# george-gca/sr-pytorch-lightning

Measured on AMD Instinct MI355X. Metric: SR training throughput, LR patches/s (48x48 LR x4, fwd+bwd+Adam), higher is better.
Workload: dtype bf16; 1 GPU; edsr_baseline x4, 48x48 LR patches, batch 256/GPU, train step (L1 + Adam); global_batch=256, parallelism=dp1, hip_graph=full

## Files before the change

include/srk.h:

```cpp
#ifndef SRK_H
#define SRK_H

#include <stdint.h>

#ifdef __cplusplus
extern "C" {
#endif

typedef void* srk_stream_t;

enum { SRK_BF16 = 0, SRK_F16 = 1, SRK_F32 = 2 };

enum {
  SRK_E_BADARG = -1,
  SRK_E_NODEV = -2
};

enum {
  SRK_OUT_NHWC = 0,
  SRK_OUT_NHWC_PS = 1,
  SRK_OUT_PLANAR = 2
};

typedef struct {
// ... 175 lines not shown
  const float* src; void* dst; int dst_pitch, dst_coff;
  int N, C, H, W;
  int Cstore; int ps_r; float scale; int dtype;
} srk_to_nhwc_args;
int srk_nchw_to_nhwc(const srk_to_nhwc_args* a, srk_stream_t stream);

typedef struct {
  const void* src; int src_pitch, src_coff; float* dst;
  int N, C, H, W; int dtype;
} srk_to_nchw_args;
int srk_nhwc_to_nchw(const srk_to_nchw_args* a, srk_stream_t stream);

int srk_ca_splits(int N, int HW);
typedef struct {
  const void* t; int t_pitch, t_coff;
  const void* u; int u_pitch, u_coff;
  float* sums;
  int N, HW, C; int dtype;
} srk_ca_pool_args;
int srk_ca_pool(const srk_ca_pool_args* a, srk_stream_t stream);

typedef struct {
  const void* t; int t_pitch, t_coff;
  const void* res; int res_pitch, res_coff;
  const float* sums;
  const float* w1; const float* b1; const float* w2; const float* b2;
  float* s_out; float* z_out;
  void* out; int out_pitch, out_coff;
  int N, HW, C, Cr; int dtype;
  int sums_rows;
} srk_ca_apply_args;
int srk_ca_apply(const srk_ca_apply_args* a, srk_stream_t stream);

typedef struct {
  const void* g; int g_pitch, g_coff;
  const float* gsum;
  const float* sums; const float* s; const float* z;
  const float* w1; const float* w2;
  float* dw1; float* db1; float* dw2; float* db2;
  void* gt; int gt_pitch, gt_coff;
  int N, HW, C, Cr; int dtype;
  int sums_rows, gsum_rows;
} srk_ca_bwd_args;
int srk_ca_bwd_apply(const srk_ca_bwd_args* a, srk_stream_t stream);
typedef struct { const float* src; float* dst; int n; int k; } srk_rowsum_job;
int srk_rowsum_group(const srk_rowsum_job* table_dev, int njobs, int max_k, srk_stream_t stream);

typedef struct {
  const uint8_t* lr; const uint8_t* hr;
  int lr_h, lr_w, hr_h, hr_w;
  int top, left;
  int rot;
  int hflip, vflip;
} srk_patch_desc;
typedef struct {
  const srk_patch_desc* table; int N; int C; int patch_lr; int scale;
  float* lr_out;
  float* hr_out;
} srk_patch_args;
int srk_sample_patches(const srk_patch_args* a, srk_stream_t stream);

typedef struct {
  const float* sr; const float* hr;
  int N, C, H, W;
  int luma;
  int shave;
  double* sse;
} srk_sse_args;
int srk_image_sse(const srk_sse_args* a, srk_stream_t stream);

typedef struct srk_l1_args {
  const float* sr;
  const float* hr;
  long long n;
  signed char* sign;
  double* partial;
  const float* gout;
  float scale;
  float* grad;
} srk_l1_args;
int srk_l1_blocks(long long n);
int srk_l1_loss_fwd(const srk_l1_args* a, srk_stream_t stream);
int srk_l1_loss_bwd(const srk_l1_args* a, srk_stream_t stream);
int srk_l1_loss_mean(const double* partial, int nb, long long n, float* out, srk_stream_t stream);

#define SRK_FLIP_TABLE_FLOATS 176
#define SRK_FLIP_ADJ_CHANNELS 7
typedef struct srk_flip_args {
  const float* sr;
  const float* hr;
  int N, H, W;
  const float* table;
  double* partial;
  float* err;
  float* adj;
  const float* gout;
  float scale;
  float* grad;
} srk_flip_args;
int srk_flip_blocks(int N, int H, int W);
int srk_flip_fwd(const srk_flip_args* a, srk_stream_t stream);
int srk_flip_bwd(const srk_flip_args* a, srk_stream_t stream);
int srk_flip_mean(const double* partial, int nb, long long n, float* out, srk_stream_t stream);

typedef struct srk_haarpsi_args {
  const float* sr;
  const float* hr;
  int N, C, H, W;
  double* partial;
  float* planes;
  float* stats;
  float* loss;
  float* index;
  const float* gout;
  float* grad;
} srk_haarpsi_args;
int srk_haarpsi_tiles(int N, int H, int W);
int srk_haarpsi_fwd(const srk_haarpsi_args* a, srk_stream_t stream);
int srk_haarpsi_finalize(const srk_haarpsi_args* a, srk_stream_t stream);
int srk_haarpsi_bwd(const srk_haarpsi_args* a, srk_stream_t stream);

typedef struct srk_ssim_loss_args {
  const float* sr;
  const float* hr;
  int N, C, H, W;
  double* partial;
  float* loss;
  const float* gout;
  float* grad;
} srk_ssim_loss_args;
int srk_ssim_loss_tiles(int N, int C, int H, int W);
int srk_ssim_loss_fwd(const srk_ssim_loss_args* a, srk_stream_t stream);
int srk_ssim_loss_finalize(const srk_ssim_loss_args* a, srk_stream_t stream);
int srk_ssim_loss_bwd(const srk_ssim_loss_args* a, srk_stream_t stream);

typedef struct srk_ms_ssim_loss_args {
  const float* sr;
  const float* hr;
  int N, C, H, W;
  float* workspace;
  double* partials;
  float* table;
  float* loss;
  const float* gout;
  float* gwork;
  float* grad;
} srk_ms_ssim_loss_args;
long long srk_ms_ssim_loss_workspace_bytes(int N, int C, int H, int W);
int srk_ms_ssim_loss_tiles(int N, int C, int H, int W, int* first);
int srk_ms_ssim_loss_fwd(const srk_ms_ssim_loss_args* a, srk_stream_t stream);
int srk_ms_ssim_loss_finalize(const srk_ms_ssim_loss_args* a, srk_stream_t stream);
int srk_ms_ssim_loss_bwd(const srk_ms_ssim_loss_args* a, srk_stream_t stream);

typedef struct srk_gmsd_args {
  const float* sr;
  const float* hr;
  int N, C, H, W;
  double* partial;
  float* stats;
  float* loss;
  const float* gout;
  float* grad;
} srk_gmsd_args;
int srk_gmsd_tiles(int N, int C, int H, int W);
int srk_gmsd_fwd(const srk_gmsd_args* a, srk_stream_t stream);
int srk_gmsd_finalize(const srk_gmsd_args* a, srk_stream_t stream);
// ... 225 lines not shown
```

sr-pytorch-lightning_amd/_lib.py:

```python
import ctypes as C
import os

_HERE = os.path.dirname(os.path.abspath(__file__))
EXACT_RELU = os.environ.get("SRK_EXACT_RELU") == "1"
LIB_PATH = os.environ.get("SRK_LIB_PATH") or os.path.join(_HERE, "libsrk_gfx950_exact.so" if EXACT_RELU else "libsrk_gfx950.so")

SRK_BF16, SRK_F16, SRK_F32 = 0, 1, 2
OUT_NHWC, OUT_NHWC_PS, OUT_PLANAR = 0, 1, 2

_p, _i, _f = C.c_void_p, C.c_int, C.c_float


class PackArgs(C.Structure):
    _fields_ = [("w", _p), ("bias", _p), ("wpk", _p), ("bias_pk", _p),
                ("Cout", _i), ("Cin", _i), ("KH", _i), ("KW", _i),
                ("KinP", _i), ("CoutP", _i), ("dgrad", _i), ("ps_r", _i), ("dtype", _i), ("rows_layout", _i)]


class ConvArgs(C.Structure):
    _fields_ = [("x", _p), ("x_pitch", _i), ("x_coff", _i), ("x_ps", _i),
                ("N", _i), ("H", _i), ("W", _i), ("Cin", _i),
                ("wpk", _p), ("bias", _p), ("CoutP", _i), ("Cout", _i), ("KH", _i), ("KW", _i),
                ("relu", _i), ("scale", _f),
                ("res", _p), ("res_pitch", _i), ("res_coff", _i),
# ... 97 lines not shown
                ("dwp", _p), ("dbp", _p), ("nslabs", _i), ("dtype", _i), ("cout_real", _i)]


class WgradFinArgs(C.Structure):
    _fields_ = [("dwp", _p), ("dbp", _p), ("nslabs", _i), ("dw", _p), ("db", _p),
                ("Cout", _i), ("Cin", _i), ("KH", _i), ("KW", _i), ("CinP", _i), ("CoutP", _i),
                ("ps_r", _i), ("scale", _f), ("accumulate", _i)]


class ProjArgs(C.Structure):
    _fields_ = [("x", _p), ("x_pitch", _i), ("out", _p), ("out_pitch", _i), ("wpk", _p), ("bias", _p),
                ("N", _i), ("H", _i), ("W", _i), ("dtype", _i), ("slope", _p), ("slope_stride", _i), ("pre", _p), ("pre_pitch", _i)]


class ProjPackJob(C.Structure):
    _fields_ = [("w4", _p), ("wpk", _p)]


class ProjWgradArgs(C.Structure):
    _fields_ = [("xh", _p), ("xh_pitch", _i), ("g", _p), ("g_pitch", _i), ("scratch", _p), ("dw", _p), ("accumulate", _i),
                ("N", _i), ("H", _i), ("W", _i), ("dtype", _i), ("db", _p), ("bias_side", _i), ("db_accumulate", _i)]


class UnfoldArgs(C.Structure):
    _fields_ = [("x", _p), ("sub", _p), ("dst", _p), ("dst_pitch", _i), ("dst_coff", _i),
                ("N", _i), ("Cin", _i), ("H", _i), ("W", _i), ("KH", _i), ("KW", _i), ("Kstore", _i), ("dtype", _i)]


class ToNhwcArgs(C.Structure):
    _fields_ = [("src", _p), ("dst", _p), ("dst_pitch", _i), ("dst_coff", _i),
                ("N", _i), ("C", _i), ("H", _i), ("W", _i), ("Cstore", _i), ("ps_r", _i), ("scale", _f), ("dtype", _i)]


class ToNchwArgs(C.Structure):
    _fields_ = [("src", _p), ("src_pitch", _i), ("src_coff", _i), ("dst", _p),
                ("N", _i), ("C", _i), ("H", _i), ("W", _i), ("dtype", _i)]


class CaPoolArgs(C.Structure):
    _fields_ = [("t", _p), ("t_pitch", _i), ("t_coff", _i), ("u", _p), ("u_pitch", _i), ("u_coff", _i),
                ("sums", _p), ("N", _i), ("HW", _i), ("C", _i), ("dtype", _i)]


class CaApplyArgs(C.Structure):
    _fields_ = [("t", _p), ("t_pitch", _i), ("t_coff", _i), ("res", _p), ("res_pitch", _i), ("res_coff", _i),
                ("sums", _p), ("w1", _p), ("b1", _p), ("w2", _p), ("b2", _p), ("s_out", _p), ("z_out", _p),
                ("out", _p), ("out_pitch", _i), ("out_coff", _i),
                ("N", _i), ("HW", _i), ("C", _i), ("Cr", _i), ("dtype", _i), ("sums_rows", _i)]


class CaBwdArgs(C.Structure):
    _fields_ = [("g", _p), ("g_pitch", _i), ("g_coff", _i), ("gsum", _p), ("sums", _p), ("s", _p), ("z", _p),
                ("w1", _p), ("w2", _p), ("dw1", _p), ("db1", _p), ("dw2", _p), ("db2", _p),
                ("gt", _p), ("gt_pitch", _i), ("gt_coff", _i),
                ("N", _i), ("HW", _i), ("C", _i), ("Cr", _i), ("dtype", _i), ("sums_rows", _i), ("gsum_rows", _i)]


class PatchDesc(C.Structure):
    _fields_ = [("lr", _p), ("hr", _p), ("lr_h", _i), ("lr_w", _i), ("hr_h", _i), ("hr_w", _i),
                ("top", _i), ("left", _i), ("rot", _i), ("hflip", _i), ("vflip", _i)]


class PatchArgs(C.Structure):
    _fields_ = [("table", _p), ("N", _i), ("C", _i), ("patch_lr", _i), ("scale", _i), ("lr_out", _p), ("hr_out", _p)]


class SseArgs(C.Structure):
    _fields_ = [("sr", _p), ("hr", _p), ("N", _i), ("C", _i), ("H", _i), ("W", _i), ("luma", _i), ("shave", _i), ("sse", _p)]


class SsimArgs(C.Structure):
    _fields_ = [("x", _p), ("y", _p), ("N", _i), ("C", _i), ("H", _i), ("W", _i), ("pool", _i),
                ("sigma", _f), ("k1", _f), ("k2", _f), ("sums", _p)]


class MsSsimArgs(C.Structure):
    _fields_ = [("x", _p), ("y", _p), ("workspace", _p), ("partials", _p), ("out", _p), ("N", _i), ("C", _i), ("H", _i), ("W", _i),
                ("sigma", _f), ("k1", _f), ("k2", _f), ("w0", _f), ("w1", _f), ("w2", _f), ("w3", _f), ("w4", _f)]


class L1Args(C.Structure):
    _fields_ = [("sr", _p), ("hr", _p), ("n", C.c_longlong), ("sign", _p), ("partial", _p), ("gout", _p),
                ("scale", _f), ("grad", _p)]


class FlipArgs(C.Structure):
    _fields_ = [("sr", _p), ("hr", _p), ("N", _i), ("H", _i), ("W", _i), ("table", _p), ("partial", _p), ("err", _p), ("adj", _p),
                ("gout", _p), ("scale", _f), ("grad", _p)]


class HaarpsiArgs(C.Structure):
    _fields_ = [("sr", _p), ("hr", _p), ("N", _i), ("C", _i), ("H", _i), ("W", _i), ("partial", _p), ("planes", _p), ("stats", _p), ("loss", _p),
                ("index", _p), ("gout", _p), ("grad", _p)]


class SsimLossArgs(C.Structure):
    _fields_ = [("sr", _p), ("hr", _p), ("N", _i), ("C", _i), ("H", _i), ("W", _i), ("partial", _p), ("loss", _p), ("gout", _p),
                ("grad", _p)]


class GmsdArgs(C.Structure):
    _fields_ = [("sr", _p), ("hr", _p), ("N", _i), ("C", _i), ("H", _i), ("W", _i), ("partial", _p), ("stats", _p), ("loss", _p),
                ("gout", _p), ("grad", _p)]


class MsSsimLossArgs(C.Structure):
    _fields_ = [("sr", _p), ("hr", _p), ("N", _i), ("C", _i), ("H", _i), ("W", _i), ("workspace", _p), ("partials", _p), ("table", _p),
                ("loss", _p), ("gout", _p), ("gwork", _p), ("grad", _p)]


class UnfoldNhwcArgs(C.Structure):
    _fields_ = [("x", _p), ("x_pitch", _i), ("x_coff", _i), ("cols", _p), ("cols_pitch", _i),
                ("N", _i), ("H", _i), ("W", _i), ("C", _i), ("K", _i), ("stride", _i), ("pad", _i), ("Ho", _i), ("Wo", _i), ("dtype", _i)]


class FoldNhwcArgs(C.Structure):
    _fields_ = [("cols", _p), ("cols_pitch", _i), ("bias", _p), ("out", _p), ("out_pitch", _i), ("out_coff", _i),
                ("N", _i), ("Hi", _i), ("Wi", _i), ("C", _i), ("K", _i), ("stride", _i), ("pad", _i), ("Ho", _i), ("Wo", _i), ("dtype", _i)]


class ChanStatsArgs(C.Structure):
    _fields_ = [("x", _p), ("x_pitch", _i), ("x_coff", _i), ("y", _p), ("y_pitch", _i), ("y_coff", _i),
                ("P", C.c_longlong), ("C", _i), ("mode", _i), ("partial", _p), ("dtype", _i), ("shift", _p), ("shift_out", _p),
                ("gate_out", _p), ("gate_pitch", _i), ("slope", _p), ("slope_stride", _i),
                ("gate_a", _p), ("gate_d", _p), ("partial2", _p)]


class ChanApplyArgs(C.Structure):
    _fields_ = [("x", _p), ("x_pitch", _i), ("x_coff", _i), ("y", _p), ("y_pitch", _i), ("y_coff", _i),
                ("z", _p), ("z_pitch", _i), ("z_coff", _i), ("a", _p), ("b", _p), ("d", _p),
                ("slope", _p), ("slope_stride", _i), ("post_prelu", _i), ("out", _p), ("out_pitch", _i), ("out_coff", _i),
                ("P", C.c_longlong), ("C", _i), ("dtype", _i), ("gate_a", _p), ("gate_d", _p)]


class HrTailArgs(C.Structure):
    _fields_ = [("wt", _p), ("bt", _p), ("wu", _p), ("bu", _p), ("O", _i), ("C", _i), ("Ci", _i),
                ("weff", _p), ("beff", _p), ("wedge", _p), ("bedge", _p), ("wcor", _p), ("bcor", _p),
                ("x", _p), ("x_pitch", _i), ("N", _i), ("H", _i), ("W", _i), ("dtype", _i),
                ("out", _p), ("g", _p), ("dx", _p), ("dx_pitch", _i),
                ("eedge", _p), ("e0", _p), ("ecor", _p), ("k0", _p), ("scratch", _p),
                ("r", _p), ("r0", _p), ("dwt", _p), ("dbt", _p), ("dwu", _p), ("dbu", _p)]


class TileDesc(C.Structure):
    _fields_ = [("y0", _i), ("x0", _i), ("id", _i), ("oy", _i), ("ox", _i), ("oh", _i), ("ow", _i), ("pad_", _i)]


class TileArgs(C.Structure):
    _fields_ = [("src", _p), ("dst", _p), ("table", _p), ("N", _i), ("C", _i), ("H", _i), ("W", _i), ("th", _i), ("tw", _i),
                ("scale", _i), ("max_oh", _i), ("max_ow", _i), ("accumulate", _i), ("weight", _f)]


LAUNCHERS = {
    "srk_pack_conv_weights": PackArgs,
    "srk_conv2d": ConvArgs,
    "srk_conv_pair": ConvPairArgs,
    "srk_pw_pack": PwPackArgs,
    "srk_pw_forward": PwArgs,
    "srk_pw_backward": PwBwdArgs,
    "srk_pw_wgrad": PwWgradArgs,
    "srk_adam_step": AdamArgs,
    "srk_ranger_step": RangerArgs,
    "srk_sgd_step": SgdArgs,
    "srk_rmsprop_step": RmspropArgs,
    "srk_chan_finalize": ChanFinalizeArgs,
    "srk_conv2d_wgrad": WgradArgs,
    "srk_wgrad_finalize": WgradFinArgs,
    "srk_unfold_nchw": UnfoldArgs,
    "srk_nchw_to_nhwc": ToNhwcArgs,
    "srk_nhwc_to_nchw": ToNchwArgs,
    "srk_ca_pool": CaPoolArgs,
    "srk_ca_apply": CaApplyArgs,
    "srk_ca_bwd_apply": CaBwdArgs,
    "srk_sample_patches": PatchArgs,
    "srk_image_sse": SseArgs,
    "srk_image_ssim": SsimArgs,
    "srk_ms_ssim": MsSsimArgs,
    "srk_l1_loss_fwd": L1Args,
    "srk_l1_loss_bwd": L1Args,
    "srk_flip_fwd": FlipArgs,
    "srk_flip_bwd": FlipArgs,
    "srk_haarpsi_fwd": HaarpsiArgs,
    "srk_haarpsi_finalize": HaarpsiArgs,
    "srk_haarpsi_bwd": HaarpsiArgs,
    "srk_ssim_loss_fwd": SsimLossArgs,
    "srk_ssim_loss_finalize": SsimLossArgs,
    "srk_ssim_loss_bwd": SsimLossArgs,
    "srk_ms_ssim_loss_fwd": MsSsimLossArgs,
    "srk_ms_ssim_loss_finalize": MsSsimLossArgs,
    "srk_ms_ssim_loss_bwd": MsSsimLossArgs,
    "srk_gmsd_fwd": GmsdArgs,
    "srk_gmsd_finalize": GmsdArgs,
    "srk_gmsd_bwd": GmsdArgs,
    "srk_unfold_nhwc": UnfoldNhwcArgs,
    "srk_fold_nhwc": FoldNhwcArgs,
    "srk_chan_stats": ChanStatsArgs,
    "srk_chan_apply": ChanApplyArgs,
    "srk_proj_down": ProjArgs,
    "srk_proj_up": ProjArgs,
    "srk_proj_wgrad": ProjWgradArgs,
    "srk_hrtail_collapse": HrTailArgs,
    "srk_hrtail_edge_fwd": HrTailArgs,
    "srk_hrtail_edge_bwd_x": HrTailArgs,
    "srk_hrtail_edge_bwd_w": HrTailArgs,
    "srk_hrtail_expand": HrTailArgs,
    "srk_tile_gather": TileArgs,
    "srk_tile_place": TileArgs,
}
OTHER_SYMBOLS = ("srk_conv_tile", "srk_last_error", "srk_version", "srk_device_cus", "srk_wgrad_slabs",
                 "srk_pack_conv_weights_group", "srk_l1_blocks", "srk_wgrad_group_ok", "srk_wgrad_group_job_bytes",
                 "srk_wgrad_group_plan", "srk_conv2d_wgrad_group", "srk_wgrad_finalize_group", "srk_upload_small", "srk_upload_prepare", "srk_upload_eager", "srk_upload_fence", "srk_ca_splits", "srk_chan_stats_blocks",
                 "srk_conv_pair_tiles", "srk_rowsum_group", "srk_pw_shape_ok", "srk_pw_pack_bytes", "srk_pw_pack_group", "srk_weight_norm_group", "srk_pw_wgrad_ranges", "srk_l1_loss_mean", "srk_chan_stats_finalize", "srk_pack_group_tiles", "srk_pack_conv_weights_group_tiled",
                 "srk_proj_pack", "srk_proj_pack_bytes", "srk_proj_wgrad_scratch_floats", "srk_proj_pack_group", "srk_wgrad_slab_cout",
                 "srk_hrtail_scratch_floats", "srk_adam_step_scaled", "srk_adam_check_scaled", "srk_adam_update_scaled", "srk_loss_scale_update", "srk_conv_bits_ok",
                 "srk_ranger_step_scaled", "srk_ranger_check_scaled", "srk_ranger_update_scaled",
                 "srk_sgd_step_scaled", "srk_sgd_check_scaled", "srk_sgd_update_scaled",
                 "srk_rmsprop_step_scaled", "srk_rmsprop_check_scaled", "srk_rmsprop_update_scaled",
                 "srk_conv_trunk", "srk_conv_trunk_ok", "srk_flip_blocks", "srk_flip_mean",
                 "srk_ms_ssim_workspace_bytes", "srk_ms_ssim_tiles", "srk_haarpsi_tiles", "srk_ssim_loss_tiles",
                 "srk_ms_ssim_loss_workspace_bytes", "srk_ms_ssim_loss_tiles", "srk_gmsd_tiles")

_lib = None


def load():
    global _lib
    if _lib is not None:
        return _lib
    if not os.path.exists(LIB_PATH):
        raise RuntimeError(
            f"{LIB_PATH} is missing: build it with `python __graft_entry__.py` "
            "(hipcc --offload-arch=gfx950).  There is no CPU fallback for the HIP path.")
    lib = C.CDLL(LIB_PATH)
    older = bool(os.environ.get("SRK_LIB_PATH"))

    class _Absent:
        def __init__(self, name):
            self.name = name
            self.argtypes = self.restype = None

        def __call__(self, *a, **k):
            raise RuntimeError(f"{self.name} is not exported by {LIB_PATH} (an older build loaded through SRK_LIB_PATH)")

    if older:
        for name in list(LAUNCHERS) + list(OTHER_SYMBOLS):
            if not hasattr(lib, name):
                setattr(lib, name, _Absent(name))
    for name, st in LAUNCHERS.items():
        fn = getattr(lib, name)
        fn.argtypes = [C.POINTER(st), C.c_void_p]
        fn.restype = C.c_int
    lib.srk_conv_tile.argtypes = [C.c_int]
    lib.srk_conv_tile.restype = C.c_int
    lib.srk_conv_pair_tiles.argtypes = [C.c_int, C.c_int, C.c_int]
    lib.srk_conv_pair_tiles.restype = C.c_int
    lib.srk_wgrad_slabs.argtypes = [C.POINTER(WgradArgs)]
    lib.srk_wgrad_slabs.restype = C.c_int
    lib.srk_wgrad_slab_cout.argtypes = [C.POINTER(WgradArgs)]
    lib.srk_wgrad_slab_cout.restype = C.c_int
    lib.srk_pack_conv_weights_group.argtypes = [C.c_void_p, C.c_int, C.c_void_p]
    lib.srk_pack_conv_weights_group.restype = C.c_int
    lib.srk_pack_group_tiles.argtypes = [C.c_void_p, C.c_int, C.c_void_p]
# ... 123 lines not shown
```

sr-pytorch-lightning_amd/csrc/data.hip:

```cpp
#include "srk_common.h"

namespace {

__device__ __forceinline__ void src_of(int y, int x, int S, int rot, int hf, int vf, int& i, int& j) {
  if (vf) y = S - 1 - y;
  if (hf) x = S - 1 - x;
  switch (rot & 3) {
    case 0: i = y; j = x; break;
    case 1: i = x; j = S - 1 - y; break;
    case 2: i = S - 1 - y; j = S - 1 - x; break;
    default: i = S - 1 - x; j = y; break;
  }
}

__global__ __launch_bounds__(256) void patch_kernel(const srk_patch_args a) {
  const int n = blockIdx.y;
  const srk_patch_desc d = a.table[n];
  const int pl = a.patch_lr, ph = a.patch_lr * a.scale;
  const int npl = pl * pl, nph = ph * ph;
  for (int t = blockIdx.x * blockDim.x + threadIdx.x; t < npl + nph; t += gridDim.x * blockDim.x) {
    const bool is_hr = t >= npl;
    const int q = is_hr ? t - npl : t;
    const int S = is_hr ? ph : pl;
    const int y = q / S, x = q - y * S;
// ... 101 lines not shown
#pragma unroll
    for (int k = 0; k < 11; ++k) {
      const float w = g[k];
#pragma unroll
      for (int q = 0; q < 5; ++q) m[q] += w * Hm[q][r + k][c];
    }
    const float c1 = a.k1 * a.k1, c2 = a.k2 * a.k2;
    const float sxx = m[2] - m[0] * m[0], syy = m[3] - m[1] * m[1], sxy = m[4] - m[0] * m[1];
    const float cs = (2.f * sxy + c2) / (sxx + syy + c2);
    const float ss = (2.f * m[0] * m[1] + c1) / (m[0] * m[0] + m[1] * m[1] + c1) * cs;
    acc = (double)ss;
  }
#pragma unroll
  for (int off = 32; off > 0; off >>= 1) acc += __shfl_down(acc, off, 64);
  if ((tid & 63) == 0) red[tid >> 6] = acc;
  __syncthreads();
  if (tid == 0) atomicAdd(a.sums + plane, red[0] + red[1] + red[2] + red[3]);
}

constexpr int L1_BLOCKS_MAX = 2048;
__global__ __launch_bounds__(256) void l1_fwd_kernel(const srk_l1_args a) {
  __shared__ double red[4];
  const long long n4 = a.n >> 2;
  double acc = 0.0;
  for (long long i = (long long)blockIdx.x * 256 + threadIdx.x; i < n4; i += (long long)gridDim.x * 256) {
    const float4 s = reinterpret_cast<const float4*>(a.sr)[i], h = reinterpret_cast<const float4*>(a.hr)[i];
    const float d[4] = {s.x - h.x, s.y - h.y, s.z - h.z, s.w - h.w};
    unsigned pk = 0;
    float t = 0.f;
#pragma unroll
    for (int k = 0; k < 4; ++k) {
      t += fabsf(d[k]);
      const int sg = (d[k] > 0.f) - (d[k] < 0.f);
      pk |= (unsigned)(sg & 0xff) << (8 * k);
    }
    acc += (double)t;
    reinterpret_cast<unsigned*>(a.sign)[i] = pk;
  }
  if (blockIdx.x == 0 && threadIdx.x < (a.n & 3)) {
    const long long i = (n4 << 2) + threadIdx.x;
    const float d = a.sr[i] - a.hr[i];
    acc += (double)fabsf(d);
    a.sign[i] = (signed char)((d > 0.f) - (d < 0.f));
  }
#pragma unroll
  for (int off = 32; off > 0; off >>= 1) acc += __shfl_down(acc, off, 64);
  if ((threadIdx.x & 63) == 0) red[threadIdx.x >> 6] = acc;
  __syncthreads();
  if (threadIdx.x == 0) a.partial[blockIdx.x] = red[0] + red[1] + red[2] + red[3];
}
__global__ __launch_bounds__(64) void l1_mean_kernel(const double* __restrict__ partial, int nb, long long n, float* __restrict__ out) {
  double t = 0.0;
  int i = threadIdx.x;
  for (; i + 64 * 7 < nb; i += 64 * 8) {
    double v[8];
#pragma unroll
    for (int k = 0; k < 8; ++k) v[k] = partial[i + 64 * k];
#pragma unroll
    for (int k = 0; k < 8; ++k) t += v[k];
  }
  for (; i < nb; i += 64) t += partial[i];
#pragma unroll
  for (int off = 32; off > 0; off >>= 1) t += __shfl_down(t, off, 64);
  if (threadIdx.x == 0) *out = (float)(t / (double)n);
}
__global__ __launch_bounds__(256) void l1_bwd_kernel(const srk_l1_args a) {
  const float g = *a.gout * a.scale;
  const long long n4 = a.n >> 2;
  for (long long i = (long long)blockIdx.x * 256 + threadIdx.x; i < n4; i += (long long)gridDim.x * 256) {
    const unsigned pk = reinterpret_cast<const unsigned*>(a.sign)[i];
    float4 o;
    o.x = g * (float)(signed char)(pk & 0xff);
    o.y = g * (float)(signed char)((pk >> 8) & 0xff);
    o.z = g * (float)(signed char)((pk >> 16) & 0xff);
    o.w = g * (float)(signed char)(pk >> 24);
    reinterpret_cast<float4*>(a.grad)[i] = o;
  }
  if (blockIdx.x == 0 && threadIdx.x < (a.n & 3)) {
    const long long i = (n4 << 2) + threadIdx.x;
    a.grad[i] = g * (float)a.sign[i];
  }
}

}

extern "C" int srk_l1_blocks(long long n) {
  const long long b = (n / 4 + 255) / 256;
  return (int)(b < 1 ? 1 : (b > L1_BLOCKS_MAX ? L1_BLOCKS_MAX : b));
}
extern "C" int srk_l1_loss_fwd(const srk_l1_args* a, srk_stream_t stream) {
  SRK_CHECK_ARG(a && a->sr && a->hr && a->sign && a->partial && a->n > 0, "srk_l1_loss_fwd: null pointer / empty");
  SRK_CHECK_ARG(((uintptr_t)a->sr | (uintptr_t)a->hr | (uintptr_t)a->sign) % 16 == 0, "srk_l1_loss_fwd: 16-byte alignment");
  hipLaunchKernelGGL(l1_fwd_kernel, dim3(srk_l1_blocks(a->n)), dim3(256), 0, reinterpret_cast<hipStream_t>(stream), *a);
  SRK_LAUNCH_CHECK();
  return 0;
}
extern "C" int srk_l1_loss_mean(const double* partial, int nb, long long n, float* out, srk_stream_t stream) {
  SRK_CHECK_ARG(partial && out && nb > 0 && n > 0, "srk_l1_loss_mean: null pointer / empty");
  hipLaunchKernelGGL(l1_mean_kernel, dim3(1), dim3(64), 0, reinterpret_cast<hipStream_t>(stream), partial, nb, n, out);
  SRK_LAUNCH_CHECK();
  return 0;
}
extern "C" int srk_l1_loss_bwd(const srk_l1_args* a, srk_stream_t stream) {
  SRK_CHECK_ARG(a && a->sign && a->gout && a->grad && a->n > 0, "srk_l1_loss_bwd: null pointer / empty");
  SRK_CHECK_ARG(((uintptr_t)a->grad | (uintptr_t)a->sign) % 16 == 0, "srk_l1_loss_bwd: 16-byte alignment");
  hipLaunchKernelGGL(l1_bwd_kernel, dim3(srk_l1_blocks(a->n)), dim3(256), 0, reinterpret_cast<hipStream_t>(stream), *a);
  SRK_LAUNCH_CHECK();
  return 0;
}

extern "C" int srk_image_ssim(const srk_ssim_args* a, srk_stream_t stream) {
  SRK_CHECK_ARG(a && a->x && a->y && a->sums, "srk_image_ssim: null pointer");
  SRK_CHECK_ARG(a->N > 0 && a->C > 0 && (long long)a->N * a->C <= 65535 && a->pool >= 1 && a->sigma > 0.f, "srk_image_ssim: bad sizes");
  const int Hp = a->H / a->pool, Wp = a->W / a->pool;
  SRK_CHECK_ARG(Hp >= 11 && Wp >= 11, "srk_image_ssim: image %dx%d (pooled %dx%d) is smaller than the 11x11 window", a->H, a->W, Hp, Wp);
  const int tilesX = (Wp - 10 + 15) / 16, tilesY = (Hp - 10 + 15) / 16;
  hipLaunchKernelGGL(ssim_kernel, dim3((unsigned)(tilesX * tilesY), (unsigned)(a->N * a->C)), dim3(256), 0,
                     reinterpret_cast<hipStream_t>(stream), *a, tilesX, Hp, Wp);
  SRK_LAUNCH_CHECK();
  return 0;
}

extern "C" int srk_sample_patches(const srk_patch_args* a, srk_stream_t stream) {
  SRK_CHECK_ARG(a && a->table && a->lr_out && a->hr_out, "srk_sample_patches: null pointer");
  SRK_CHECK_ARG(a->N > 0 && a->N <= 65535 && a->C > 0 && a->C <= 4 && a->patch_lr > 0 && a->scale > 0, "srk_sample_patches: bad sizes");
  const int total = a->patch_lr * a->patch_lr * (1 + a->scale * a->scale);
  int gx = (total + 255) / 256;
  if (gx > 64) gx = 64;
  hipLaunchKernelGGL(patch_kernel, dim3(gx, a->N), dim3(256), 0, reinterpret_cast<hipStream_t>(stream), *a);
  SRK_LAUNCH_CHECK();
  return 0;
}

extern "C" int srk_image_sse(const srk_sse_args* a, srk_stream_t stream) {
  SRK_CHECK_ARG(a && a->sr && a->hr && a->sse, "srk_image_sse: null pointer");
  SRK_CHECK_ARG(a->N > 0 && a->N <= 65535 && a->C > 0 && a->H > 2 * a->shave && a->W > 2 * a->shave && a->shave >= 0, "srk_image_sse: bad sizes");
  SRK_CHECK_ARG(!a->luma || a->C == 3, "srk_image_sse: luma needs 3 channels");
  const long long npix = (long long)(a->H - 2 * a->shave) * (a->W - 2 * a->shave);
  long long gx = (npix + 255) / 256;
  if (gx > 512) gx = 512;
  hipLaunchKernelGGL(sse_kernel, dim3((unsigned)gx, a->N), dim3(256), 0, reinterpret_cast<hipStream_t>(stream), *a);
  SRK_LAUNCH_CHECK();
  return 0;
}
```

sr-pytorch-lightning_amd/ops.py:

```python
import weakref

import torch

from . import _lib as L
from .packing import *
from .packing import _DT, _TLS, _f32c, _group_for, _knob, _need_gpu, _ptr, _roundup, _stream, _tok


def _pitch(t):
    n, h, w, c = t.shape
    p = t.stride(2) if w > 1 else (t.stride(1) if h > 1 else (t.stride(0) if n > 1 else c))
    if w > 1 and h > 1:
        assert t.stride(1) == w * p, "NHWC view must be dense in W"
    if h > 1 and n > 1:
        assert t.stride(0) == h * w * p, "NHWC view must be dense in H"
    assert c == 1 or t.stride(3) == 1, "channels must be innermost"
    return p


_ADDR_LIMIT = 0x7fff0000


def _batch_chunks(n, *tensors):
    worst = 0
# ... 317 lines not shown
        ctx.cfg = (ps_r, b is not None, res is not None)
        ctx.wb = (w, b)
        ctx.pg = _tok()
        return out

    @staticmethod
    def backward(ctx, g):
        x, w = ctx.saved_tensors
        ps_r, has_b, has_res = ctx.cfg
        n, h, wd, cinp = x.shape
        cout, cin, k, _ = w.shape
        dy = to_nhwc(g, x.dtype, ps_r=ps_r)
        gx = gw = gb = None
        if ctx.needs_input_grad[0]:
            pkd = pack_conv(w, None, x.dtype, dgrad=True, token=ctx.pg)
            gx = torch.empty_like(x)
            conv_raw(dy, pkd, N=n, H=h, W=wd, Cin=dy.shape[3], Cout=cinp, out=gx, use_bias=False)
        if ctx.needs_input_grad[1] or ctx.needs_input_grad[2]:
            gw, gb = wgrad(x, dy, wparam=ctx.wb[0], bparam=ctx.wb[1], N=n, H=h, W=wd, Cin=cinp, Cout=dy.shape[3], k=k,
                           w_shape=tuple(w.shape), want_bias=has_b)
            gw = gw if ctx.needs_input_grad[1] else None
        return gx, gw, gb, (g if has_res else None), None, None


def tail_conv(x, w, b, *, res=None, post_add=None, ps_r=0):
    return TailConvFn.apply(x, w, b, res, post_add, int(ps_r))


class SkipConvFn(torch.autograd.Function):

    @staticmethod
    def forward(ctx, x, w, b, sub, ps_r, dtype):
        _need_gpu(x)
        cout, cin, k, _ = w.shape
        n, c, h, wd = x.shape
        r = ps_r if ps_r > 1 else 1
        xu = unfold_raw(x, sub, k, dtype)
        pk = _pack_head(w, b, dtype)
        out = torch.empty((n, cout // (r * r), h * r, wd * r), dtype=torch.float32, device=x.device)
        conv_raw(xu, pk, N=n, H=h, W=wd, Cin=xu.shape[3], Cout=cout, out=out, out_mode=L.OUT_PLANAR, ps_r=ps_r)
        ctx.save_for_backward(xu, w)
        ctx.cfg = (ps_r, b is not None)
        return out

    @staticmethod
    def backward(ctx, g):
        xu, w = ctx.saved_tensors
        ps_r, has_b = ctx.cfg
        n, h, wd, kp = xu.shape
        gw = gb = None
        if ctx.needs_input_grad[1] or ctx.needs_input_grad[2]:
            dy = to_nhwc(g, xu.dtype, ps_r=ps_r)
            gw, gb = wgrad_raw(xu, dy, N=n, H=h, W=wd, Cin=kp, Cout=dy.shape[3], k=1, w_shape=tuple(w.shape),
                               want_bias=has_b)
            gw = gw if ctx.needs_input_grad[1] else None
        return None, gw, gb, None, None, None


def skip_conv(x, w, b, sub, ps_r, dtype):
    return SkipConvFn.apply(x, w, b, sub, int(ps_r), dtype)


_HR_COLLAPSE = _knob("SRK_NO_HR_COLLAPSE", "0") != "1"


def hr_tail_ok(x, wu, wt, ps_r):
    if not _HR_COLLAPSE or int(ps_r) != 2 or x.dtype not in (torch.bfloat16, torch.float16):
        return False
    cu, ci, ku, _ = wu.shape
    o, c, kt, _ = wt.shape
    if ku != 3 or kt != 3 or cu != 4 * c or ci != 64 or x.shape[3] != 64 or not 1 <= o <= 4:
        return False
    n, h, w, _ = x.shape
    return n > 0 and max(h, w) <= 512 and x.numel() * 2 < _ADDR_LIMIT and n * o * 4 * h * w < (1 << 31)


def _hr_bufs(o, ci, dev):
    f32 = torch.float32
    return dict(weff=torch.empty((4 * o, ci, 5, 5), dtype=f32, device=dev), beff=torch.empty(4 * o, dtype=f32, device=dev),
                wedge=torch.empty((4, 2 * o, ci, 5), dtype=f32, device=dev), bedge=torch.empty((4, 2 * o), dtype=f32, device=dev),
                wcor=torch.empty((4, o, ci), dtype=f32, device=dev), bcor=torch.empty((4, o), dtype=f32, device=dev))


class HrTailFn(torch.autograd.Function):

    @staticmethod
    def _args(x, wu, bu, wt, bt, bufs, **kw):
        n, h, w, _ = x.shape
        o, c = wt.shape[0], wt.shape[1]
        return L.HrTailArgs(wt=wt.data_ptr(), bt=_ptr(bt), wu=wu.data_ptr(), bu=_ptr(bu), O=o, C=c, Ci=wu.shape[1],
                            weff=bufs["weff"].data_ptr(), beff=bufs["beff"].data_ptr(), wedge=bufs["wedge"].data_ptr(),
                            bedge=bufs["bedge"].data_ptr(), wcor=bufs["wcor"].data_ptr(), bcor=bufs["bcor"].data_ptr(),
                            x=x.data_ptr(), x_pitch=_pitch(x), N=n, H=h, W=w, dtype=_DT[x.dtype], **kw)

    @staticmethod
    def forward(ctx, x, wu, bu, wt, bt, post_add):
        _need_gpu(x)
        n, h, w, ci = x.shape
        o = wt.shape[0]
        dev, f32 = x.device, torch.float32
        wu_, wt_ = _f32c(wu), _f32c(wt)
        bu_, bt_ = (None if bu is None else _f32c(bu)), (None if bt is None else _f32c(bt))
        bufs = _hr_bufs(o, ci, dev)
        L.call("srk_hrtail_collapse", HrTailFn._args(x, wu_, bu_, wt_, bt_, bufs), _stream())
        pk = pack_conv(bufs["weff"], bufs["beff"], x.dtype, cache=False)
        out = torch.empty((n, o, 2 * h, 2 * w), dtype=f32, device=dev)
        conv_raw(x, pk, N=n, H=h, W=w, Cin=ci, Cout=4 * o, out=out, out_mode=L.OUT_PLANAR, ps_r=2, post_add=post_add)
        L.call("srk_hrtail_edge_fwd", HrTailFn._args(x, wu_, bu_, wt_, bt_, bufs, out=out.data_ptr()), _stream())
        ctx.save_for_backward(x, wu_, wt_, *( [bu_] if bu_ is not None else []))
        ctx.has = (bu is not None, bt is not None)
        ctx.bufs = bufs
        ctx.wb = (wu, bu, wt, bt)
        return out

    @staticmethod
    def backward(ctx, g):
        x, wu_, wt_ = ctx.saved_tensors[:3]
        has_bu, has_bt = ctx.has
        bu_ = ctx.saved_tensors[3] if has_bu else None
        bufs = ctx.bufs
        n, h, w, ci = x.shape
        o, c = wt_.shape[0], wt_.shape[1]
        dev, f32 = x.device, torch.float32
        g = _f32c(g)
        st = _stream()
        g12 = to_nhwc(g, x.dtype, ps_r=2)
        need_x = ctx.needs_input_grad[0]
        need_w = any(ctx.needs_input_grad[1:5])
        gx = None
        if need_x:
            pkd = pack_conv(bufs["weff"], None, x.dtype, dgrad=True, cache=False)
            gx = torch.empty_like(x)
            conv_raw(g12, pkd, N=n, H=h, W=w, Cin=g12.shape[3], Cout=ci, out=gx, use_bias=False)
            L.call("srk_hrtail_edge_bwd_x", HrTailFn._args(x, wu_, bu_, wt_, None, bufs, g=g.data_ptr(), dx=gx.data_ptr(), dx_pitch=_pitch(gx)), st)
        gwu = gbu = gwt = gbt = None
        if need_w:
            r, r0 = wgrad_raw(x, g12, N=n, H=h, W=w, Cin=ci, Cout=g12.shape[3], k=5, w_shape=(4 * o, ci, 5, 5), want_bias=True)
            red = dict(eedge=torch.empty((4, 2 * o, ci, 5), dtype=f32, device=dev), e0=torch.empty((4, 2 * o), dtype=f32, device=dev),
                       ecor=torch.empty((4, o, ci), dtype=f32, device=dev), k0=torch.empty((4, o), dtype=f32, device=dev))
            scratch = torch.empty(int(L.load().srk_hrtail_scratch_floats(n, ci)), dtype=f32, device=dev)
            ptrs = {k: v.data_ptr() for k, v in red.items()}
            L.call("srk_hrtail_edge_bwd_w", HrTailFn._args(x, wu_, bu_, wt_, None, bufs, g=g.data_ptr(), scratch=scratch.data_ptr(), **ptrs), st)
            pu, pbu, pt, pbt = ctx.wb
            gwu, gwt = (route(p, shape, dev, slice=p.dtype == f32, buffer=True).out for p, shape in ((pu, tuple(wu_.shape)), (pt, tuple(wt_.shape))))
            gbu = route(pbu, (4 * c,), dev, slice=pbu.dtype == f32, buffer=True).out if has_bu else None
            gbt = route(pbt, (o,), dev, slice=pbt.dtype == f32, buffer=True).out if has_bt else None
            L.call("srk_hrtail_expand", HrTailFn._args(x, wu_, bu_, wt_, None, bufs, r=r.data_ptr(), r0=r0.data_ptr(), dwt=gwt.data_ptr(),
                                                       dbt=_ptr(gbt), dwu=gwu.data_ptr(), dbu=_ptr(gbu), **ptrs), st)
        return gx, gwu, gbu, gwt, gbt, None


def hr_tail(x, wu, bu, wt, bt, *, post_add=None):
    return HrTailFn.apply(x, wu, bu, wt, bt, post_add)


class ConvChainFn(torch.autograd.Function):

    @staticmethod
    def forward(ctx, x, scale, relus, *params):
        _need_gpu(x)
        L_ = len(relus)
        ws, bs = params[0::2], params[1::2]
        n, h, wd, _ = x.shape
        acts = [x]
        bits = []
        a = x
        paired = L_ == 2 and tuple(relus) == (True, False) and pair_ok(x, ws[0], ws[1])
        if paired:
            y1 = torch.empty_like(x)
            a = conv_pair_raw(x, pack_conv(ws[0], bs[0], x.dtype), pack_conv(ws[1], bs[1], x.dtype), out=torch.empty_like(x),
                              relu_mid=True, mid=y1, scale_out=scale, res=x)
            acts.append(y1)
        for i in range(0 if paired else L_):
            w = ws[i]
            cout, cin, k, _ = w.shape
            pk = pack_conv(w, bs[i], x.dtype)
            out = torch.empty((n, h, wd, pad16(cout)), dtype=x.dtype, device=x.device)
            last = i == L_ - 1
            conv_raw(a, pk, N=n, H=h, W=wd, Cin=a.shape[3], Cout=out.shape[3], out=out, relu=relus[i],
                     scale=scale if last else 1.0, res=x if last else None,
                     relu_bits="want" if (relus[i] and not last and ctx.needs_input_grad[0]) else None)
            a = out
            if not last:
                acts.append(a)
                bits.append(out.__dict__.pop("_srk_bits", None))
        ctx.bits = bits
        ctx.save_for_backward(*acts, *ws)
        ctx.cfg = (scale, tuple(relus), tuple(b is not None for b in bs))
        ctx.wb = (tuple(ws), tuple(bs))
        ctx.pg = _tok()
        return a

    @staticmethod
    def backward(ctx, g):
        scale, relus, has_b = ctx.cfg
        L_ = len(relus)
        acts, ws = ctx.saved_tensors[:L_], ctx.saved_tensors[L_:]
        g = g.contiguous()
        n, h, wd, _ = g.shape
        grads = [None] * (2 * L_)
        dy = g
        paired = L_ == 2 and relus == (True, False) and pair_ok(g, ws[0], ws[1])
        if paired:
            x, y1 = acts
            g1 = torch.empty_like(g)
            gx = conv_pair_raw(g, pack_conv(ws[1], None, g.dtype, dgrad=True, token=ctx.pg),
                               pack_conv(ws[0], None, g.dtype, dgrad=True, token=ctx.pg), out=torch.empty_like(g),
                               scale_mid=scale, mask=y1, mid=g1, res=g, use_bias=False)
            for i, (a_in, d, sc) in enumerate(((x, g1, 1.0), (y1, g, scale))):
# ... 754 lines not shown
```

sr-pytorch-lightning_amd/ops_metrics.py:

```python
import ctypes
import os

import torch

from . import _lib as L
from .ops import _f32c, _need_gpu, _stream


def image_sse(sr, hr, *, luma=False, shave=0):
    _need_gpu(sr)
    n, c, h, w = sr.shape
    s32, h32 = _f32c(sr), _f32c(hr)
    sse = torch.zeros(n, dtype=torch.float64, device=sr.device)
    a = L.SseArgs(sr=s32.data_ptr(), hr=h32.data_ptr(), N=n, C=c, H=h, W=w, luma=int(luma), shave=int(shave), sse=sse.data_ptr())
    L.call("srk_image_sse", a, _stream())
    count = (h - 2 * shave) * (w - 2 * shave) * (1 if luma else c)
    return sse, count


def psnr(sr, hr, *, luma=False, shave=0, eps=1e-8):
    sse, count = image_sse(sr, hr, luma=luma, shave=shave)
    return (10.0 * torch.log10(1.0 / (sse / count + eps))).mean().float()


def ssim(x, y, *, sigma=1.5, k1=0.01, k2=0.03):
    _need_gpu(x)
    xs, ys = _f32c(x), _f32c(y)
    n, c, h, w = xs.shape
    f = max(1, round(min(h, w) / 256))
    sums = torch.zeros(n * c, dtype=torch.float64, device=xs.device)
    a = L.SsimArgs(x=xs.data_ptr(), y=ys.data_ptr(), N=n, C=c, H=h, W=w, pool=f, sigma=float(sigma), k1=float(k1), k2=float(k2),
                   sums=sums.data_ptr())
    L.call("srk_image_ssim", a, _stream())
    count = (h // f - 10) * (w // f - 10)
    return (sums / count).mean().float()


MS_SSIM_WEIGHTS = (0.0448, 0.2856, 0.3001, 0.2363, 0.1333)
MS_SSIM_MIN_SIZE = (11 - 1) * 2 ** (len(MS_SSIM_WEIGHTS) - 1) + 1


def ms_ssim_check(x, y):
    if x.dim() != 4 or tuple(x.shape) != tuple(y.shape):
        raise ValueError(f"ms_ssim expects two N x C x H x W tensors of one shape, got {tuple(x.shape)} and {tuple(y.shape)}")
    if min(x.shape[-2:]) < MS_SSIM_MIN_SIZE:
        raise ValueError(f"Invalid size of the input images, expected at least {MS_SSIM_MIN_SIZE}x{MS_SSIM_MIN_SIZE}.")


def _ms_ssim_launch(x, y, sigma, k1, k2):
    _need_gpu(x)
    ms_ssim_check(x, y)
    xs, ys = _f32c(x), _f32c(y)
    n, c, h, w = xs.shape
    lib = L.load()
    first = (ctypes.c_int * (len(MS_SSIM_WEIGHTS) + 1))()
    tiles = lib.srk_ms_ssim_tiles(h, w, first)
    pyr = lib.srk_ms_ssim_workspace_bytes(n, c, h, w)
    if tiles <= 0 or pyr < 0:
        raise RuntimeError(f"srk_ms_ssim refused the sizes {tuple(xs.shape)}")
    ws = torch.empty(pyr + n * c * tiles * 16, dtype=torch.uint8, device=xs.device)
    out = torch.empty((), dtype=torch.float32, device=xs.device)
    w0, w1, w2, w3, w4 = MS_SSIM_WEIGHTS
    a = L.MsSsimArgs(x=xs.data_ptr(), y=ys.data_ptr(), workspace=ws.data_ptr(), partials=ws.data_ptr() + pyr, out=out.data_ptr(),
                     N=n, C=c, H=h, W=w, sigma=float(sigma), k1=float(k1), k2=float(k2), w0=w0, w1=w1, w2=w2, w3=w3, w4=w4)
    L.call("srk_ms_ssim", a, _stream())
    return out, ws[pyr:].view(torch.float64).view(n * c, tiles, 2), list(first)


def ms_ssim(x, y, *, sigma=1.5, k1=0.01, k2=0.03):
    return _ms_ssim_launch(x, y, sigma, k1, k2)[0]


def ms_ssim_levels(x, y, *, sigma=1.5, k1=0.01, k2=0.03):
    out, part, first = _ms_ssim_launch(x, y, sigma, k1, k2)
    n, c, h, w = x.shape
    hs, ws = [h], [w]
    for _ in range(len(MS_SSIM_WEIGHTS) - 1):
        p = max(hs[-1] % 2, ws[-1] % 2)
        hs.append((hs[-1] + p) // 2)
        ws.append((ws[-1] + p) // 2)
    cs, ss = [], []
    for k in range(len(MS_SSIM_WEIGHTS)):
        s = part[:, first[k]:first[k + 1]].sum(dim=1) / ((hs[k] - 10) * (ws[k] - 10))
        ss.append(s[:, 0].view(n, c))
        cs.append(s[:, 1].view(n, c))
    return out, torch.stack(cs), torch.stack(ss)


class L1LossFn(torch.autograd.Function):

    @staticmethod
    def forward(ctx, sr, hr):
        _need_gpu(sr)
        s, h = _f32c(sr), _f32c(hr)
        n = s.numel()
        sign = torch.empty(n, dtype=torch.int8, device=s.device)
        nb = L.load().srk_l1_blocks(n)
        partial = torch.empty(nb, dtype=torch.float64, device=s.device)
        a = L.L1Args(sr=s.data_ptr(), hr=h.data_ptr(), n=n, sign=sign.data_ptr(), partial=partial.data_ptr(), gout=0, scale=0.0, grad=0)
        L.call("srk_l1_loss_fwd", a, _stream())
        ctx.save_for_backward(sign)
        ctx.shape = tuple(sr.shape)
        out = torch.empty((), dtype=torch.float32, device=s.device)
        L.check(L.load().srk_l1_loss_mean(partial.data_ptr(), nb, n, out.data_ptr(), _stream()), "srk_l1_loss_mean")
        return out

    @staticmethod
    def backward(ctx, g):
        (sign,) = ctx.saved_tensors
        n = sign.numel()
        gout = g.detach().float().contiguous()
        grad = torch.empty(ctx.shape, dtype=torch.float32, device=sign.device)
        a = L.L1Args(sr=0, hr=0, n=n, sign=sign.data_ptr(), partial=0, gout=gout.data_ptr(), scale=1.0 / n, grad=grad.data_ptr())
        L.call("srk_l1_loss_bwd", a, _stream())
        return grad, None


def l1_loss(sr, hr):
    if hr.requires_grad or sr.numel() == 0:
        return torch.nn.functional.l1_loss(sr, hr)
    return L1LossFn.apply(sr, hr)
```

Before: 47340 LR patches/s.

## Fuse L1 loss backward directly into HR tail pixel-shuffle NHWC gradient layout

Adds a kernel that turns the L1 sign buffer straight into the bf16/f16 pixel-shuffled NHWC gradient the HR tail backward consumes, plus an fp32 border ring. The L1 backward hands autograd a zero placeholder, and the tail backward swaps in the precomputed buffers. This skips writing a full fp32 gradient and the separate to_nhwc conversion pass. It relies on autograd task ids and placeholder identity checks, and falls back to the old path when hooks or retained grads are present.

Measured after the change: 47740 LR patches/s (median of 6 runs). Within noise of the previous version (+0.9%).

```diff
diff --git a/include/srk.h b/include/srk.h
--- a/include/srk.h
+++ b/include/srk.h
@@ -281,6 +281,16 @@
 int srk_l1_blocks(long long n);
 int srk_l1_loss_fwd(const srk_l1_args* a, srk_stream_t stream);
 int srk_l1_loss_bwd(const srk_l1_args* a, srk_stream_t stream);
+typedef struct {
+  const signed char* sign;
+  const float* gout;
+  float scale;
+  int N, C, H, W;
+  void* dst; int dst_pitch;
+  float* ring;
+  int dtype;
+} srk_l1_tail_args;
+int srk_l1_loss_bwd_tail(const srk_l1_tail_args* a, srk_stream_t stream);
 int srk_l1_loss_mean(const double* partial, int nb, long long n, float* out, srk_stream_t stream);
 
 #define SRK_FLIP_TABLE_FLOATS 176
diff --git a/sr-pytorch-lightning_amd/_lib.py b/sr-pytorch-lightning_amd/_lib.py
--- a/sr-pytorch-lightning_amd/_lib.py
+++ b/sr-pytorch-lightning_amd/_lib.py
@@ -203,6 +203,11 @@
 class L1Args(C.Structure):
     _fields_ = [("sr", _p), ("hr", _p), ("n", C.c_longlong), ("sign", _p), ("partial", _p), ("gout", _p),
                 ("scale", _f), ("grad", _p)]
+
+
+class L1TailArgs(C.Structure):
+    _fields_ = [("sign", _p), ("gout", _p), ("scale", _f), ("N", _i), ("C", _i), ("H", _i), ("W", _i),
+                ("dst", _p), ("dst_pitch", _i), ("ring", _p), ("dtype", _i)]
 
 
 class FlipArgs(C.Structure):
@@ -299,6 +304,7 @@
     "srk_ms_ssim": MsSsimArgs,
     "srk_l1_loss_fwd": L1Args,
     "srk_l1_loss_bwd": L1Args,
+    "srk_l1_loss_bwd_tail": L1TailArgs,
     "srk_flip_fwd": FlipArgs,
     "srk_flip_bwd": FlipArgs,
     "srk_haarpsi_fwd": HaarpsiArgs,
diff --git a/sr-pytorch-lightning_amd/csrc/data.hip b/sr-pytorch-lightning_amd/csrc/data.hip
--- a/sr-pytorch-lightning_amd/csrc/data.hip
+++ b/sr-pytorch-lightning_amd/csrc/data.hip
@@ -207,6 +207,58 @@
   }
 }
 
+template <int DT> __global__ __launch_bounds__(256) void l1_bwd_tail_kernel(const srk_l1_tail_args a) {
+  typedef DTraits<DT> Tr;
+  const float g = *a.gout * a.scale;
+  const int C = a.C, H2 = a.H, W2 = a.W, H = H2 >> 1, W = W2 >> 1;
+  const size_t plane = (size_t)H2 * W2;
+  typename Tr::elem* const dst = reinterpret_cast<typename Tr::elem*>(a.dst);
+  const long long total = (long long)a.N * H * W;
+  for (long long t = (long long)blockIdx.x * 256 + threadIdx.x; t < total; t += (long long)gridDim.x * 256) {
+    const int x = (int)(t % W);
+    const long long q = t / W;
+    const int y = (int)(q % H), n = (int)(q / H);
+    float v[16];
+#pragma unroll
+    for (int c = 0; c < 4; ++c) {
+#pragma unroll
+      for (int i = 0; i < 2; ++i) {
+        float lo = 0.f, hi = 0.f;
+        if (c < C) {
+          const unsigned w = *reinterpret_cast<const unsigned short*>(a.sign + ((size_t)n * C + c) * plane + (size_t)(2 * y + i) * W2 + 2 * x);
+          lo = g * (float)(signed char)(w & 0xff);
+          hi = g * (float)(signed char)(w >> 8);
+        }
+        v[c * 4 + i * 2] = lo; v[c * 4 + i * 2 + 1] = hi;
+      }
+    }
+    typename Tr::elem* const o = dst + (size_t)t * a.dst_pitch;
+#pragma unroll
+    for (int h = 0; h < 2; ++h) {
+      i32x4 raw;
+      raw.x = (int)pack2<DT>(v[8 * h + 0], v[8 * h + 1]); raw.y = (int)pack2<DT>(v[8 * h + 2], v[8 * h + 3]);
+      raw.z = (int)pack2<DT>(v[8 * h + 4], v[8 * h + 5]); raw.w = (int)pack2<DT>(v[8 * h + 6], v[8 * h + 7]);
+      *reinterpret_cast<i32x4*>(o + 8 * h) = raw;
+    }
+    if (a.ring) {
+      const bool top = y == 0, bot = y == H - 1, left = x == 0, right = x == W - 1;
+      if (top || bot || left || right) {
+#pragma unroll
+        for (int c = 0; c < 4; ++c) {
+          if (c >= C) break;
+#pragma unroll
+          for (int i = 0; i < 2; ++i) {
+            float* const r = a.ring + ((size_t)n * C + c) * plane + (size_t)(2 * y + i) * W2 + 2 * x;
+            const bool row = (top && i == 0) || (bot && i == 1);
+            if (row || left) r[0] = v[c * 4 + i * 2];
+            if (row || right) r[1] = v[c * 4 + i * 2 + 1];
+          }
+        }
+      }
+    }
+  }
+}
+
 }
 
 extern "C" int srk_l1_blocks(long long n) {
@@ -230,6 +282,22 @@
   SRK_CHECK_ARG(a && a->sign && a->gout && a->grad && a->n > 0, "srk_l1_loss_bwd: null pointer / empty");
   SRK_CHECK_ARG(((uintptr_t)a->grad | (uintptr_t)a->sign) % 16 == 0, "srk_l1_loss_bwd: 16-byte alignment");
   hipLaunchKernelGGL(l1_bwd_kernel, dim3(srk_l1_blocks(a->n)), dim3(256), 0, reinterpret_cast<hipStream_t>(stream), *a);
+  SRK_LAUNCH_CHECK();
+  return 0;
+}
+
+extern "C" int srk_l1_loss_bwd_tail(const srk_l1_tail_args* a, srk_stream_t stream) {
+  SRK_CHECK_ARG(a && a->sign && a->gout && a->dst, "srk_l1_loss_bwd_tail: null pointer");
+  SRK_CHECK_ARG(a->N > 0 && a->C >= 1 && a->C <= 4 && a->H >= 2 && a->W >= 2 && a->H % 2 == 0 && a->W % 2 == 0,
+                "srk_l1_loss_bwd_tail: N=%d C=%d H=%d W=%d (1..4 channels, even image sizes)", a->N, a->C, a->H, a->W);
+  SRK_CHECK_ARG(a->dst_pitch >= 16 && a->dst_pitch % 8 == 0 && (uintptr_t)a->dst % 16 == 0 && (uintptr_t)a->sign % 2 == 0,
+                "srk_l1_loss_bwd_tail: dst_pitch=%d / alignment", a->dst_pitch);
+  SRK_CHECK_ARG(a->dtype == SRK_BF16 || a->dtype == SRK_F16, "srk_l1_loss_bwd_tail: dtype %d (16-bit only)", a->dtype);
+  const long long b = ((long long)a->N * (a->H / 2) * (a->W / 2) + 255) / 256;
+  const dim3 grid((unsigned)(b > 8192 ? 8192 : b)), block(256);
+  hipStream_t st = reinterpret_cast<hipStream_t>(stream);
+  if (a->dtype == SRK_BF16) hipLaunchKernelGGL(l1_bwd_tail_kernel<SRK_BF16>, grid, block, 0, st, *a);
+  else hipLaunchKernelGGL(l1_bwd_tail_kernel<SRK_F16>, grid, block, 0, st, *a);
   SRK_LAUNCH_CHECK();
   return 0;
 }
diff --git a/sr-pytorch-lightning_amd/ops.py b/sr-pytorch-lightning_amd/ops.py
--- a/sr-pytorch-lightning_amd/ops.py
+++ b/sr-pytorch-lightning_amd/ops.py
@@ -423,6 +423,55 @@
                 wcor=torch.empty((4, o, ci), dtype=f32, device=dev), bcor=torch.empty((4, o), dtype=f32, device=dev))
 
 
+_L1_TAIL = _knob("SRK_NO_L1_TAIL", "0") != "1"
+_ZEROS = {}
+
+
+class TailGrad:
+    __slots__ = ("shape", "dtype", "g12", "ring", "placeholder", "l1", "task")
+
+    def __init__(self, shape, dtype):
+        self.shape, self.dtype = tuple(shape), dtype
+        self.g12 = self.ring = self.placeholder = self.l1 = self.task = None
+
+    def filled(self):
+        return self.g12 is not None and self.task == torch._C._current_graph_task_id()
+
+    def fill_l1(self, sign, gout, scale):
+        if self.filled():
+            return None
+        self.task = torch._C._current_graph_task_id()
+        n, c, h2, w2 = self.shape
+        dev = sign.device
+        self.g12 = torch.empty((n, h2 // 2, w2 // 2, 16), dtype=self.dtype, device=dev)
+        self.ring = torch.empty(self.shape, dtype=torch.float32, device=dev)
+        a = L.L1TailArgs(sign=sign.data_ptr(), gout=gout.data_ptr(), scale=scale, N=n, C=c, H=h2, W=w2, dst=self.g12.data_ptr(),
+                         dst_pitch=16, ring=self.ring.data_ptr(), dtype=_DT[self.dtype])
+        L.call("srk_l1_loss_bwd_tail", a, _stream())
+        self.l1 = (sign, gout, scale)
+        zero = _ZEROS.get(dev)
+        if zero is None:
+            zero = torch.zeros((), dtype=torch.float32, device=dev)
+            if not torch.cuda.is_current_stream_capturing():
+                _ZEROS[dev] = zero
+        self.placeholder = zero.expand(self.shape)
+        return self.placeholder
+
+    def take(self, g):
+        ok = self.filled()
+        g12, ring, ph, l1 = self.g12, self.ring, self.placeholder, self.l1
+        self.g12 = self.ring = self.placeholder = self.l1 = self.task = None
+        if not ok:
+            return None
+        if g is ph and g.data_ptr() == ph.data_ptr():
+            return g12, ring, None
+        sign, gout, scale = l1
+        grad = torch.empty(self.shape, dtype=torch.float32, device=sign.device)
+        a = L.L1Args(sr=0, hr=0, n=sign.numel(), sign=sign.data_ptr(), partial=0, gout=gout.data_ptr(), scale=scale, grad=grad.data_ptr())
+        L.call("srk_l1_loss_bwd", a, _stream())
+        return None, None, grad
+
+
 class HrTailFn(torch.autograd.Function):
 
     @staticmethod
@@ -452,6 +501,9 @@
         ctx.has = (bu is not None, bt is not None)
         ctx.bufs = bufs
         ctx.wb = (wu, bu, wt, bt)
+        ctx.tail = None
+        if _L1_TAIL:
+            ctx.tail = out.__dict__["_srk_tail"] = TailGrad(out.shape, x.dtype)
         return out
 
     @staticmethod
@@ -463,9 +515,15 @@
         n, h, w, ci = x.shape
         o, c = wt_.shape[0], wt_.shape[1]
         dev, f32 = x.device, torch.float32
-        g = _f32c(g)
         st = _stream()
-        g12 = to_nhwc(g, x.dtype, ps_r=2)
+        taken = ctx.tail.take(g) if ctx.tail is not None else None
+        if taken is not None and taken[0] is not None:
+            g12, g = taken[0], taken[1]
+        else:
+            g = _f32c(g)
+            if taken is not None:
+                g = taken[2].add_(g)
+            g12 = to_nhwc(g, x.dtype, ps_r=2)
         need_x = ctx.needs_input_grad[0]
         need_w = any(ctx.needs_input_grad[1:5])
         gx = None
diff --git a/sr-pytorch-lightning_amd/ops_metrics.py b/sr-pytorch-lightning_amd/ops_metrics.py
--- a/sr-pytorch-lightning_amd/ops_metrics.py
+++ b/sr-pytorch-lightning_amd/ops_metrics.py
@@ -1,9 +1,11 @@
 import ctypes
 import os
+import weakref as _weakref
 
 import torch
 
 from . import _lib as L
+from . import ops as _ops
 from .ops import _f32c, _need_gpu, _stream
 
 
@@ -101,6 +103,10 @@
         L.call("srk_l1_loss_fwd", a, _stream())
         ctx.save_for_backward(sign)
         ctx.shape = tuple(sr.shape)
+        ctx.tail = ctx.sr_ref = None
+        tail = sr.__dict__.get("_srk_tail") if _ops._L1_TAIL else None
+        if tail is not None and tail.shape == ctx.shape and s.data_ptr() == sr.data_ptr():
+            ctx.tail, ctx.sr_ref = tail, _weakref.ref(sr)
         out = torch.empty((), dtype=torch.float32, device=s.device)
         L.check(L.load().srk_l1_loss_mean(partial.data_ptr(), nb, n, out.data_ptr(), _stream()), "srk_l1_loss_mean")
         return out
@@ -110,6 +116,14 @@
         (sign,) = ctx.saved_tensors
         n = sign.numel()
         gout = g.detach().float().contiguous()
+        tail = ctx.tail
+        if tail is not None:
+            sr = ctx.sr_ref()
+            if sr is not None and (sr.retains_grad or sr._backward_hooks):
+                tail = None
+        placeholder = tail.fill_l1(sign, gout, 1.0 / n) if tail is not None else None
+        if placeholder is not None:
+            return placeholder, None
         grad = torch.empty(ctx.shape, dtype=torch.float32, device=sign.device)
         a = L.L1Args(sr=0, hr=0, n=n, sign=sign.data_ptr(), partial=0, gout=gout.data_ptr(), scale=1.0 / n, grad=grad.data_ptr())
         L.call("srk_l1_loss_bwd", a, _stream())
```
